# filodb/FiloDB

Measured on AMD Instinct MI355X. Metric: samples/sec scanned+aggregated, 1M series rate()[5m], higher is better.
Workload: dtype f64; 1 GPU; 1M counter series 1h@15s, rate()[5m] step=15s; series_per_gpu=1000000, windows=241, payload_bytes_per_gpu=886470800

## Files before the change

### filodb_amd/csrc/engine.hip

```cpp

#include <cstring>
#include <cstdio>
#include <cmath>
#include <vector>
#include <cstdlib>

#include "engine_internal.h"
#include "fast_desc.h"

struct fdb_engine {
  int device;
  hipStream_t stream;
  int32_t* dev_flag;
};

struct fdb_dataset {
  uint8_t* blob;
  uint64_t *ts_off, *val_off;
  int64_t *start_time, *end_time;
  int32_t *num_rows;
  int32_t *series_first, *series_nchunks, *group_ids;
  int32_t *series_by_group, *group_offsets;
  int32_t num_series;
  int64_t num_chunks;
  int64_t payload_bytes;
  int64_t total_samples;
  int max_group;
  int has_hist;
  int fast_ok;
  void* sums;
  uint64_t *max_off, *min_off;
  int has_mm;
  int has_sc;
  FdbFastDesc *fast_desc, *fast_desc_sc;
};

static DirSoA dir_of(const fdb_dataset_t* d, bool count_col = false) {
  return DirSoA{d->ts_off, count_col ? d->max_off : d->val_off,
                d->start_time, d->end_time, d->num_rows};
}

extern "C" fdb_engine_t* fdb_engine_create(int32_t device) {
  int count = 0;
  hipError_t e = hipGetDeviceCount(&count);
  if (e != hipSuccess || count == 0) {
    fdb_set_error("no HIP device present (hipGetDeviceCount: %s) — "
                  "filodb_amd has no CPU fallback", hipGetErrorString(e));
    return nullptr;
  }
  if (device < 0 || device >= count) { fdb_set_error("bad device %d", device); return nullptr; }
  HIP_CHECK_NULL(hipSetDevice(device));
  auto* eng = new fdb_engine();
  eng->device = device;
  if (hipStreamCreate(&eng->stream) != hipSuccess) {
    fdb_set_error("hipStreamCreate failed");
    delete eng;
    return nullptr;
  }
  if (hipMalloc(&eng->dev_flag, 4) != hipSuccess ||
      hipMemset(eng->dev_flag, 0, 4) != hipSuccess) {
    fdb_set_error("engine flag allocation failed");
    (void)hipStreamDestroy(eng->stream);
    delete eng;
    return nullptr;
  }
  return eng;
}
// ... 116 lines not shown
  };
  bool ok = upload_pad((void**)&d->blob, view.blob, (size_t)view.blob_len)
    && upload((void**)&d->ts_off, ts_off.data(), nc * 8)
    && upload((void**)&d->val_off, val_off.data(), nc * 8)
    && upload((void**)&d->start_time, st.data(), nc * 8)
    && upload((void**)&d->end_time, en.data(), nc * 8)
    && upload((void**)&d->num_rows, nr.data(), nc * 4)
    && upload((void**)&d->series_first, view.series_first, (size_t)view.num_series * 4)
    && upload((void**)&d->series_nchunks, view.series_nchunks, (size_t)view.num_series * 4)
    && upload((void**)&d->group_ids, view.group_ids, (size_t)view.num_series * 4)
    && upload((void**)&d->series_by_group, sbg.data(), sbg.size() * 4)
    && upload((void**)&d->group_offsets, goff.data(), goff.size() * 4)
    && upload((void**)&d->max_off, mx_off.data(), nc * 8)
    && upload((void**)&d->min_off, mn_off.data(), nc * 8);
  if (ok && d->fast_ok) {
    const int32_t ns = view.num_series;
    for (int col = 0; col < (d->has_sc ? 2 : 1) && d->fast_ok; col++) {
      const std::vector<uint64_t>& voff = col ? mx_off : val_off;
      std::vector<FdbFastDesc> desc((size_t)ns);
      int addressable = 1;
      #pragma omp parallel for schedule(static) reduction(&:addressable)
      for (int32_t sid = 0; sid < ns; sid++) {
        const int32_t c = view.series_first[sid];
        const bool has = view.series_nchunks[sid] >= 1;
        if (has && (((ts_off[c] | voff[c]) & 63) != 0 ||
                    ((ts_off[c] | voff[c]) >> 38) != 0)) {
          addressable = 0;
          continue;
        }
        fdb_build_fast_desc(view.blob, has ? ts_off[c] : 0, has ? voff[c] : 0,
                            has ? nr[c] : 0, &desc[(size_t)sid]);
      }
      if (!addressable) { d->fast_ok = 0; break; }
      ok = upload((void**)(col ? &d->fast_desc_sc : &d->fast_desc), desc.data(),
                  desc.size() * sizeof(FdbFastDesc));
      if (!ok) break;
    }
  }
  if (!ok) {
    fdb_set_error("device upload failed (out of HBM?)");
    fdb_dataset_destroy(d);
    return nullptr;
  }
  const char* fenv = getenv("FDB_FAST");
  const bool fast_off = fenv && atoi(fenv) == 0;
  if (has_scalar && (!d->fast_ok || fast_off)) {
    if (hipMalloc(&d->sums, (size_t)fdb_chunksum_bytes(nc)) != hipSuccess) {
      fdb_set_error("summary allocation failed (out of HBM?)");
      fdb_dataset_destroy(d);
      return nullptr;
    }
    if (fdb_launch_summaries(e->stream, d->blob, dir_of(d), nc, d->sums) != FDB_OK) {
      fdb_dataset_destroy(d);
      return nullptr;
    }
  }
  return d;
}

static bool fast_eligible(const fdb_dataset_t* d, const fdb_query_t* q) {
  const char* v = getenv("FDB_FAST");
  if (v && atoi(v) == 0) return false;
  return d->fast_ok && fdb_scan_supported(q->func_id) &&
         q->step > 0 && q->step < ((int64_t)1 << 31) && q->window >= 0;
}

static int32_t launch_scan(fdb_engine_t* e, const fdb_dataset_t* d, const fdb_query_t* q,
                           double* dev_out, double* dev_cnt, double* dev_sq,
                           bool count_col = false) {
  DirSoA dir = dir_of(d, count_col);
  int nw = fdb_num_windows(q);
  if (fast_eligible(d, q) && q->agg_id == AGG_NONE) {
    return fdb_launch_fast_scan(e->stream, d->blob,
                                count_col ? d->fast_desc_sc : d->fast_desc,
                                d->group_ids,
                                d->series_by_group, d->num_series,
                                q->start, q->step, q->window, nw,
                                q->func_id, AGG_NONE, 0,
                                dev_out, dev_cnt, dev_sq, q->_pad);
  }
  if (fdb_window_sample_supported(q->func_id)) {
    return fdb_launch_window_sample(e->stream, d->blob, dir, d->series_first,
                                    d->series_nchunks, d->num_series,
                                    q->start, q->step, q->window, nw,
                                    q->func_id, q->param, q->param2,
                                    dev_out, e->dev_flag);
  }
  if (!fdb_scan_supported(q->func_id)) {
    fdb_set_error("bad func_id %d", q->func_id);
    return FDB_ERR_BADARG;
  }
  if (!d->sums) {
    fdb_set_error("dataset has no chunk summaries (internal)");
    return FDB_ERR;
  }
  (void)dev_cnt; (void)dev_sq;
  return fdb_launch_stream_walk(e->stream, d->blob, dir, d->sums,
                                d->series_first, d->series_nchunks,
                                d->num_series, q->start, q->step, q->end,
                                q->window, nw, q->func_id, dev_out);
}

static int32_t check_windows(const fdb_query_t* q, const char* bad_nw, int* nw) {
  *nw = fdb_num_windows(q);
  if (*nw <= 0) { fdb_set_error("%s", bad_nw); return FDB_ERR_BADARG; }
  if (q->window > ((int64_t)1 << 33)) {
    fdb_set_error("window length > 2^33 ms (~99 days) unsupported");
// ... 50 lines not shown
  if (q->agg_id != AGG_NONE && !dev_cnt && !dev_cnt.alloc(out_len * 8))
    return alloc_failed("query");
  if (needs_sq) {
    if (partial) dev_sq.wrap(dev_out.get() + out_len);
    else if (!dev_sq.alloc(out_len * 8)) return alloc_failed("query");
  }
  HIP_CHECK(ev0.create());
  HIP_CHECK(ev1.create());

  const bool is_quant = q->agg_id == AGG_QUANTILE;
  if (is_quant && out_counts) {
    fdb_set_error("quantile aggregation has no partial (multi-shard) mode — "
                  "digest shipping is not implemented");
    return FDB_ERR_BADARG;
  }
  const char* fe = getenv("FDB_FUSED_GROUP");
  const bool fused = (fe && atoi(fe) == 1) && !is_quant &&
                     q->agg_id != AGG_NONE && !is_topk &&
                     nw <= 256 && fast_eligible(d, q);
  fdb_query_t qscan = *q;
  if (q->agg_id != AGG_NONE && !fused) {
    if (!per_grid.alloc((size_t)d->num_series * nw * 8)) return alloc_failed("query");
    qscan.agg_id = AGG_NONE;
  }

  auto run_once = [&]() -> int32_t {
    if (fused) {
      const bool mm = q->agg_id == AGG_MIN || q->agg_id == AGG_MAX;
      HIP_CHECK(hipMemsetAsync(dev_out.get(), mm ? 0xFF : 0, buf_len * 8, e->stream));
      HIP_CHECK(hipMemsetAsync(dev_cnt.get(), 0, out_len * 8, e->stream));
      if (dev_sq && !(needs_sq && partial))
        HIP_CHECK(hipMemsetAsync(dev_sq.get(), 0, out_len * 8, e->stream));
      return fdb_launch_fast_scan(
          e->stream, d->blob, d->fast_desc,
          d->group_ids, d->series_by_group, d->num_series,
          q->start, q->step, q->window, nw, q->func_id, q->agg_id,
          1, dev_out.get(), dev_cnt.get(), dev_sq.get(), q->_pad);
    }
    int32_t rc = launch_scan(e, d, &qscan, per_grid ? per_grid.get() : dev_out.get(),
                             per_grid ? nullptr : dev_cnt.get(), nullptr);
    if (rc != FDB_OK) return rc;
    if (is_topk)
      return fdb_launch_topk(e->stream, per_grid.get(), d->series_by_group,
                             d->group_offsets, q->num_groups, nw, kk,
                             q->agg_id == AGG_TOPK ? 1 : 0,
                             dev_out.get(), dev_cnt.get());
    if (is_quant)
      return fdb_launch_quantile_cells(e->stream, per_grid.get(),
                                       d->series_by_group, d->group_offsets,
                                       q->num_groups, nw, q->param, dev_out.get());
    if (q->agg_id != AGG_NONE)
      return fdb_launch_group_reduce(e->stream, per_grid.get(),
                                     d->series_by_group, d->group_offsets,
                                     q->num_groups, nw, q->agg_id,
                                     dev_out.get(), dev_cnt.get(), dev_sq.get());
    return FDB_OK;
  };

  int total_runs = warmup + iters;
  float ms_sum = 0;
  for (int it = 0; it < total_runs; it++) {
    bool timed = it >= warmup;
    if (timed) HIP_CHECK(hipEventRecord(ev0.get(), e->stream));
    if (int32_t rc = run_once()) return rc;
    if (timed) {
      HIP_CHECK(hipEventRecord(ev1.get(), e->stream));
      HIP_CHECK(hipEventSynchronize(ev1.get()));
// ... 223 lines not shown
```

### filodb_amd/csrc/engine_internal.h

```cpp
#ifndef FDB_ENGINE_INTERNAL_H
#define FDB_ENGINE_INTERNAL_H

#include <hip/hip_runtime.h>
#include <cstdint>

#include "chunk_format.h"
#include "scan_common.h"
#include "window_funcs.h"
#include "../../include/filodb_amd.h"

void fdb_set_error(const char* fmt, ...);
hipStream_t fdb_engine_stream(fdb_engine_t* e);

#define HIP_CHECK(expr) do { hipError_t _e = (expr); if (_e != hipSuccess) { \
  fdb_set_error("%s failed: %s", #expr, hipGetErrorString(_e)); return FDB_ERR; } } while (0)
#define HIP_CHECK_NULL(expr) do { hipError_t _e = (expr); if (_e != hipSuccess) { \
  fdb_set_error("%s failed: %s", #expr, hipGetErrorString(_e)); return nullptr; } } while (0)

template <typename T>
class DevPtr {
 public:
  DevPtr() = default;
  DevPtr(const DevPtr&) = delete;
  DevPtr& operator=(const DevPtr&) = delete;
// ... 22 lines not shown
  T* p_ = nullptr;
  bool owned_ = false;
};
using DevBuf = DevPtr<double>;

class DevEvent {
 public:
  DevEvent() = default;
  DevEvent(const DevEvent&) = delete;
  DevEvent& operator=(const DevEvent&) = delete;
  ~DevEvent() { if (ev_) (void)hipEventDestroy(ev_); }
  hipError_t create() { return hipEventCreate(&ev_); }
  hipEvent_t get() const { return ev_; }

 private:
  hipEvent_t ev_ = nullptr;
};

inline bool fdb_scan_supported(int func_id) {
  switch (func_id) {
    case FN_RATE: case FN_INCREASE: case FN_DELTA:
    case FN_SUM: case FN_COUNT: case FN_AVG: case FN_RATE_OVER_DELTA:
    case FN_MIN: case FN_MAX: case FN_STDDEV: case FN_STDVAR:
    case FN_CHANGES: case FN_LAST: case FN_PRESENT: case FN_TIMESTAMP:
    case FN_ZSCORE:
    case FN_IRATE: case FN_IDELTA: case FN_RESETS:
      return true;
    default:
      return false;
  }
}

struct FdbFastDesc;
int32_t fdb_launch_fast_scan(hipStream_t stream, const uint8_t* blob,
                             const FdbFastDesc* desc,
                             const int32_t* group_ids, const int32_t* series_by_group,
                             int num_series,
                             int64_t qstart, int64_t qstep, int64_t qwindow,
                             int num_windows, int func_id, int agg_id, int emit_group,
                             double* out, double* out_cnt, double* out_sq,
                             int phase_mask);

int32_t fdb_launch_summaries(hipStream_t stream, const uint8_t* blob, DirSoA dir,
                             int64_t num_chunks, void* sums);
int64_t fdb_chunksum_bytes(int64_t num_chunks);
int32_t fdb_launch_stream_walk(hipStream_t stream, const uint8_t* blob,
                               DirSoA dir, const void* sums,
                               const int32_t* series_first,
                               const int32_t* series_nchunks, int num_series,
                               int64_t qstart, int64_t qstep, int64_t qend,
                               int64_t qwindow, int num_windows, int func_id,
                               double* out);

bool fdb_window_sample_supported(int func_id);
int32_t fdb_launch_window_sample(hipStream_t stream, const uint8_t* blob,
                                 DirSoA dir, const int32_t* series_first,
                                 const int32_t* series_nchunks, int num_series,
                                 int64_t qstart, int64_t qstep, int64_t qwindow,
                                 int num_windows, int func_id, double param,
                                 double param2, double* out, int32_t* overflow);

int32_t fdb_launch_hist2(hipStream_t stream, const uint8_t* blob, DirSoA dir,
                         const uint64_t* max_off, const uint64_t* min_off,
                         const int32_t* series_first,
                         const int32_t* series_nchunks,
                         const int32_t* group_ids, int num_series,
                         int64_t qstart, int64_t qstep, int64_t qwindow,
                         int num_windows, int nb, int hfunc,
// ... 30 lines not shown
```

### filodb_amd/csrc/fast_desc.h

```cpp
#ifndef FDB_FAST_DESC_H
#define FDB_FAST_DESC_H

#include <cstdint>
#include <cstring>

#include "chunk_format.h"

enum { FDB_FD_CONST = 0,
       FDB_FD_PACKED = 1,
       FDB_FD_RAW64 = 2 };
enum { FDB_FD_SIGN = 1,
       FDB_FD_DROPPED = 2,
       FDB_FD_EXACT32 = 4 };

struct FdbFastDesc {
  uint32_t ts_unit;
  uint32_t val_unit;
  uint16_t n;
  uint8_t  ts_cls, ts_nbits;
  uint8_t  ts_flags, val_cls, val_nbits, val_flags;
  int64_t  ts0;
  int32_t  ts_base;
  int32_t  ts_slope;
  int64_t  val_init;
  int32_t  val_slope;
  uint32_t _pad[5];
};
static_assert(sizeof(FdbFastDesc) == 64, "one 64-byte scalar load per series");

struct FdbFdVec {
  int64_t init, first;
  int32_t slope, n;
  uint32_t payload;
  uint8_t cls, nbits, flags;
};

inline FdbFdVec fdb_fd_open(const uint8_t* p) {
  uint32_t h[8];
  memcpy(h, p, 32);
  FdbFdVec v;
  memset(&v, 0, sizeof(v));
  const uint16_t wf = (uint16_t)(h[1] & 0xffff);
  if (((h[1] >> 16) & FDB_DROP_MASK) != 0) v.flags |= FDB_FD_DROPPED;
  if (wf == FDB_WF_DDV) {
    v.cls = FDB_FD_PACKED;
    v.init = (int64_t)(((uint64_t)h[3] << 32) | h[2]);
    v.slope = (int32_t)h[4];
    const uint32_t w6 = h[6];
    v.nbits = (uint8_t)((w6 >> 16) & FDB_NBITS_MASK);
    if (((w6 >> 16) & FDB_SIGN_MASK) != 0) v.flags |= FDB_FD_SIGN;
    const int bitShift = (int)(w6 >> 24) & 0x3f;
    const int numBytes = (int)h[5];
    v.n = v.nbits
        ? ((numBytes - 4) * 8 + (bitShift != 0 ? bitShift - 8 : 0)) / v.nbits : 0;
    v.payload = FDB_DDV_OFF_INNER + FDB_PRIM_OFF_DATA;
    const bool sg = (v.flags & FDB_FD_SIGN) != 0;
    int64_t in0;
    switch (v.nbits) {
      case 32: in0 = (int32_t)h[7]; break;
// ... 7 lines not shown
    v.cls = FDB_FD_CONST;
    v.n = (int32_t)h[2];
    v.init = (int64_t)(((uint64_t)h[4] << 32) | h[3]);
    v.slope = (int32_t)h[5];
    v.first = v.init;
  } else {
    v.cls = FDB_FD_RAW64;
    v.n = ((int)h[0] - 4) / 8;
    v.nbits = 64;
    v.flags |= FDB_FD_SIGN;
    v.payload = FDB_PRIM_OFF_DATA;
    v.first = (int64_t)(((uint64_t)h[3] << 32) | h[2]);
  }
  return v;
}

inline int64_t fdb_fd_inner(const uint8_t* idata, int nbits, bool sign, int i) {
  switch (nbits) {
    case 32: { int32_t x; memcpy(&x, idata + 4 * (size_t)i, 4); return x; }
    case 16: { uint16_t u; memcpy(&u, idata + 2 * (size_t)i, 2);
               int32_t x = (int16_t)u; return sign ? x : (x & 0xffff); }
    case 8:  { int32_t x = (int8_t)idata[i]; return sign ? x : (x & 0xff); }
    case 4:  return (idata[i >> 1] >> ((i & 1) * 4)) & 0x0f;
    case 2:  return (idata[i >> 2] >> ((i & 3) * 2)) & 0x03;
  }
  return 0;
}

inline void fdb_build_fast_desc(const uint8_t* blob, uint64_t ts_off,
                                uint64_t val_off, int32_t num_rows,
                                FdbFastDesc* out) {
  FdbFastDesc d;
  memset(&d, 0, sizeof(d));
  if (num_rows > 0) {
    const FdbFdVec tv = fdb_fd_open(blob + ts_off);
    const FdbFdVec vv = fdb_fd_open(blob + val_off);
    d.ts_unit = (uint32_t)(ts_off >> 6);
    d.val_unit = (uint32_t)(val_off >> 6);
    d.ts_cls = tv.cls; d.ts_nbits = tv.nbits; d.ts_flags = tv.flags;
    d.val_cls = vv.cls; d.val_nbits = vv.nbits; d.val_flags = vv.flags;
    d.ts_slope = tv.slope;
    d.val_init = vv.init; d.val_slope = vv.slope;
    if (num_rows <= FDB_DEFAULT_MAX_ROWS && num_rows <= tv.n) {
      d.n = (uint16_t)num_rows;
      d.ts0 = tv.first;
      d.ts_base = (int32_t)(tv.init - tv.first);
      if (vv.cls == FDB_FD_PACKED && vv.n >= num_rows &&
          vv.init > -((int64_t)1 << 52) && vv.init < ((int64_t)1 << 52)) {
        const uint8_t* idata = blob + val_off + vv.payload;
        const bool sg = (vv.flags & FDB_FD_SIGN) != 0;
        bool fits = true;
        for (int i = 0; i < num_rows && fits; i++) {
          const int64_t off = (int64_t)vv.slope * i +
                              fdb_fd_inner(idata, vv.nbits, sg, i);
          fits = off >= INT32_MIN && off <= INT32_MAX;
        }
        if (fits) d.val_flags |= FDB_FD_EXACT32;
      }
    }
  }
  *out = d;
}

#endif
```

### filodb_amd/csrc/scan_fast.hip

```cpp

#include <cstddef>
#include <cstring>
#include <cmath>

#include "engine_internal.h"
#include "fast_desc.h"
#include "window_bounds.h"

#define FAST_TILE 256
#define FAST_WAVES 4
#define FAST_DROPS 32

#define K_RATE    0
#define K_PFX     1
#define K_PFX_SQ  2
#define K_MINMAX  3
#define K_CHANGES 4
#define K_LAST    5

template <int FUNC> struct FKind { static constexpr int v =
    (FUNC <= FN_DELTA) ? K_RATE :
    (FUNC == FN_SUM || FUNC == FN_AVG || FUNC == FN_COUNT ||
     FUNC == FN_RATE_OVER_DELTA) ? K_PFX :
    (FUNC == FN_STDDEV || FUNC == FN_STDVAR) ? K_PFX_SQ :
    (FUNC == FN_MIN || FUNC == FN_MAX) ? K_MINMAX :
    (FUNC == FN_CHANGES || FUNC == FN_RESETS) ? K_CHANGES :
    K_LAST; };

template <int KIND>
struct alignas(16) FWs {
  int32_t tso[FDB_DEFAULT_MAX_ROWS + 4];
  double  val[FDB_DEFAULT_MAX_ROWS];
  uint16_t cnt[(KIND == K_PFX || KIND == K_PFX_SQ || KIND == K_CHANGES)
                   ? FDB_DEFAULT_MAX_ROWS : 1];
  double  sq[KIND == K_PFX_SQ ? FDB_DEFAULT_MAX_ROWS : 1];
  double  grp[KIND == K_MINMAX ? (FDB_DEFAULT_MAX_ROWS + 7) / 8 : 1];
  int16_t dpos[KIND == K_RATE ? FAST_DROPS : 1];
  double  dcum[KIND == K_RATE ? FAST_DROPS : 1];
};

struct FDesc {
  uint32_t w[12];
  __device__ __forceinline__ int n() const { return (int)(w[2] & 0xffff); }
  __device__ __forceinline__ int ts_cls() const { return (int)((w[2] >> 16) & 0xff); }
  __device__ __forceinline__ int ts_nbits() const { return (int)(w[2] >> 24); }
  __device__ __forceinline__ int ts_flags() const { return (int)(w[3] & 0xff); }
  __device__ __forceinline__ int val_cls() const { return (int)((w[3] >> 8) & 0xff); }
  __device__ __forceinline__ int val_nbits() const { return (int)((w[3] >> 16) & 0xff); }
  __device__ __forceinline__ int val_flags() const { return (int)(w[3] >> 24); }
  __device__ __forceinline__ int64_t ts0() const {
    return (int64_t)(((uint64_t)w[5] << 32) | w[4]); }
  __device__ __forceinline__ int32_t ts_base() const { return (int32_t)w[6]; }
  __device__ __forceinline__ int32_t ts_slope() const { return (int32_t)w[7]; }
  __device__ __forceinline__ int64_t val_init() const {
    return (int64_t)(((uint64_t)w[9] << 32) | w[8]); }
  __device__ __forceinline__ int32_t val_slope() const { return (int32_t)w[10]; }
};
static_assert(offsetof(FdbFastDesc, n) == 8 && offsetof(FdbFastDesc, ts_flags) == 12 &&
              offsetof(FdbFastDesc, ts0) == 16 && offsetof(FdbFastDesc, ts_base) == 24 &&
              offsetof(FdbFastDesc, val_init) == 32 && offsetof(FdbFastDesc, val_slope) == 40,
              "FDesc's dword views follow FdbFastDesc's layout");

__device__ __forceinline__ FDesc fast_load_desc(const FdbFastDesc* desc, int s) {
  const uint4* p = reinterpret_cast<const uint4*>(desc + s);
  const uint4 a = p[0], b = p[1], c = p[2];
  return FDesc{{a.x, a.y, a.z, a.w, b.x, b.y, b.z, b.w, c.x, c.y, c.z, c.w}};
}

template <int KIND> constexpr bool needs_inv = KIND == K_PFX || KIND == K_PFX_SQ;
template <int KIND> constexpr int inv_entries =
    needs_inv<KIND> ? FDB_DEFAULT_MAX_ROWS + 2 : KIND == K_RATE ? FDB_RATE_RTAB : 0;

struct FastQuery {
  int64_t qstep, qwindow;
  double rate_scale, dur_ms;
  bool qw32;
  int rk_lim;
};

enum { PH_DECODE = 0, PH_META = 1, PH_BOUNDS = 2, PH_WINDOWS = 3 };
template <bool TIMED> struct FastTimer {
  uint64_t t[4] = {0, 0, 0, 0}, tt = 0;
  __device__ __forceinline__ void start() {
    if constexpr (TIMED) tt = __builtin_amdgcn_s_memtime();
  }
  __device__ __forceinline__ void lap(int phase) {
    if constexpr (TIMED) {
      const uint64_t now = __builtin_amdgcn_s_memtime();
      t[phase] += now - tt;
      tt = now;
    }
  }
  __device__ __forceinline__ void store(double* out, size_t gw, int lane) const {
    if constexpr (TIMED) {
      #pragma unroll
      for (int p = 0; p < 4; p++) if (lane == 0) out[gw * 4 + p] = (double)t[p];
    }
  }
};

struct FastChunk { int n; int64_t ts0; bool dropped; };

template <typename WS>
__device__ __forceinline__ FastChunk fast_decode(const FDesc& cd, const uint8_t* blob,
                                                 WS& ws, int lane) {
  const int n = cd.n();
  const int64_t ts0 = cd.ts0();
  const bool dropped = n > 0 && (cd.val_flags() & FDB_FD_DROPPED) != 0;
  if (n > 0) {
    int dl = lane;
    asm volatile("" : "+v"(dl));
    const uint8_t* tp = blob + ((size_t)cd.w[0] << 6);
    const uint8_t* vp = blob + ((size_t)cd.w[1] << 6);
    DVec tv;
    tv.wf = cd.ts_cls() == FDB_FD_PACKED ? FDB_WF_DDV
          : cd.ts_cls() == FDB_FD_CONST ? FDB_WF_DDV_CONST : FDB_WF_PRIM64;
    tv.idata = tp + (cd.ts_cls() == FDB_FD_PACKED
                         ? FDB_DDV_OFF_INNER + FDB_PRIM_OFF_DATA : FDB_PRIM_OFF_DATA);
    tv.init = ts0 + cd.ts_base();
    tv.slope = cd.ts_slope();
    tv.n = n; tv.nbits = (uint8_t)cd.ts_nbits();
    tv.sign = (cd.ts_flags() & FDB_FD_SIGN) != 0; tv.dropped = 0;
    d_decode_ts_offsets(tv, n, ts0, ws.tso, dl);
    const int vcls = cd.val_cls(), vbits = cd.val_nbits();
    const bool vsign = (cd.val_flags() & FDB_FD_SIGN) != 0;
    const bool exact32 = (cd.val_flags() & FDB_FD_EXACT32) != 0;
    const uint8_t* vdata = vp + FDB_DDV_OFF_INNER + FDB_PRIM_OFF_DATA;
    if (vcls == FDB_FD_PACKED && vbits == 8) {
      d_decode_val4<8>(vdata, vsign, cd.val_init(), cd.val_slope(), exact32,
                       n, ws.val, dl);
    } else if (vcls == FDB_FD_PACKED && vbits == 16) {
      d_decode_val4<16>(vdata, vsign, cd.val_init(), cd.val_slope(), exact32,
                        n, ws.val, dl);
    } else {
      DVec vv;
      vv.wf = vcls == FDB_FD_PACKED ? FDB_WF_DDV
            : vcls == FDB_FD_CONST ? FDB_WF_DDV_CONST : FDB_WF_PRIM64;
      vv.idata = vcls == FDB_FD_PACKED ? vdata : vp + FDB_PRIM_OFF_DATA;
      vv.init = cd.val_init(); vv.slope = cd.val_slope();
      vv.n = n; vv.nbits = (uint8_t)vbits; vv.sign = vsign; vv.dropped = dropped;
      d_decode_chunk<true>(vv, n, nullptr, ws.val, dl);
    }
  }
  return FastChunk{n, ts0, dropped};
}

template <int KIND, int FUNC, typename WS>
__device__ __forceinline__ ResetScan fast_meta(WS& ws, int n, bool dropped, int lane) {
  ResetScan rs;
  if constexpr (KIND == K_RATE) {
    if (dropped && n > 0) {
      for (int base = 0; base < n; base += 64) {
        int i = base + lane;
        double raw = (i < n) ? ws.val[i] : 0;
        double x = (i < n && !isnan(raw)) ? raw : 0;
        d_reset_scan_step<FAST_DROPS>(rs, i, i < n, x, lane, ws.dpos, ws.dcum);
// ... 24 lines not shown
      if constexpr (KIND == K_PFX_SQ) carry_sq += __shfl(sqs, 63);
    }
  }
  if constexpr (KIND == K_MINMAX) {
    for (int base = 0; base < n; base += 64) {
      int i = base + lane;
      double x = (i < n) ? ws.val[i] : NAN;
      #pragma unroll
      for (int off = 1; off < 8; off <<= 1)
        d_fold_mm<FUNC == FN_MIN>(x, __shfl_xor(x, off));
      if ((lane & 7) == 0 && i < n) ws.grp[i >> 3] = x;
    }
  }
  if constexpr (KIND == K_CHANGES) {
    int ccarry = 0;
    double carry_x = NAN;
    for (int base = 0; base < n; base += 64) {
      int i = base + lane;
      double x = (i < n) ? ws.val[i] : NAN;
      double px = __shfl_up(x, 1);
      if (lane == 0) px = carry_x;
      int ind = (i > 0 && i < n && d_pair_counts<FUNC == FN_RESETS>(x, px)) ? 1 : 0;
      int s = wave_incl_scan_i(ind, lane);
      if (i < n) ws.cnt[i] = (uint16_t)(ccarry + s);
      ccarry += __shfl(s, 63);
      carry_x = __shfl(x, 63);
    }
  }
  return rs;
}

struct WB { int s, e; int32_t t1, t2; };

template <bool SHARE>
struct FastBounds {
  const int32_t* tso;
  int n, lane, wshare;
  FastQuery q;
  FdbLin lin;
  int64_t Ae;
  int share_src;
  int s_prev;

  __device__ __forceinline__ FastBounds(const int32_t* tso_, int n_, int64_t Ae_,
                                        const FastQuery& q_, int wshare_, int lane_)
      : tso(tso_), n(n_), lane(lane_), wshare(wshare_), q(q_), Ae(Ae_),
        share_src(((lane_ - wshare_) & 63) << 2), s_prev(0) {
    const int32_t tlast = n > 0 ? tso[n - 1] : 0;
    lin.last = __builtin_amdgcn_readfirstlane(tlast);
    lin.inv_h = (n >= 2 && lin.last > 0) ? (float)(n - 1) / (float)lin.last : 0.0f;
    if constexpr (SHARE) {
      if (!fdb_windows_before_chunk(-1, q.qstep, Ae)) {
        int32_t unused;
        end_search(lane - 64, &unused, &s_prev);
      }
    }
  }
  __device__ __forceinline__ WB window_bounds(int w) const {
    WB b;
    const int64_t wEndOff = (int64_t)w * q.qstep - Ae;
    b.e = fdb_bound_e(tso, n, lin, wEndOff, &b.t2);
    b.s = fdb_bound_s(tso, n, lin, wEndOff - q.qwindow, &b.t1);
    return b;
  }
  __device__ __forceinline__ int end_search(int w, int32_t* t2, int* s_at_end) const {
    const int64_t x = (int64_t)w * q.qstep - Ae;
    int32_t t_next, unused;
    const int e = fdb_bound_core(tso, n, lin, x, t2, &t_next, nullptr);
    *s_at_end = fdb_bound_s_from_e(tso, n, lin, x, e, *t2, t_next, &unused);
    return e;
  }
  __device__ __forceinline__ WB shared_bounds(int w) {
    WB b;
    int s_cur;
    b.e = end_search(w, &b.t2, &s_cur);
    b.s = __builtin_amdgcn_ds_bpermute(share_src, lane < 64 - wshare ? s_cur : s_prev);
    s_prev = s_cur;
    b.t1 = tso[b.s];
    return b;
  }
  __device__ __forceinline__ WB calc_bounds(int k, int w, bool wok, int tn) {
    WB b = WB{1, -1, 0, 0};
    if constexpr (SHARE) {
      if (64 * k < tn) {
        const WB sb = shared_bounds(w);
        if (wok) b = sb;
      }
    } else if (wok) {
      b = window_bounds(w);
    }
    return b;
  }
};

template <int FUNC, typename WS>
__device__ __forceinline__ double fast_window_value(const WS& ws, const WB& wb, int w,
                                                    const FastChunk& ch,
                                                    const ResetScan& rs, int64_t Ae,
                                                    const FastQuery& q,
                                                    const double* inv_tab) {
  constexpr int KIND = FKind<FUNC>::v;
  const int s = wb.s, e = wb.e, n = ch.n;
  double res = NAN;
  if constexpr (KIND == K_RATE) {
    constexpr bool IS_COUNTER = (FUNC == FN_RATE || FUNC == FN_INCREASE);
    if (e > s) {
      const int t1 = wb.t1, t2 = wb.t2;
      if (t2 > t1) {
        double v1 = ws.val[s], v2 = ws.val[e];
        if (IS_COUNTER && ch.dropped) {
          if (isnan(v1)) v1 = 0;
          if (isnan(v2)) v2 = 0;
          auto row_at = [&](int j) { return ws.val[j]; };
          v1 += d_corr_at(ws.dpos, ws.dcum, rs.count, rs.dense, s, row_at);
          v2 += d_corr_at(ws.dpos, ws.dcum, rs.count, rs.dense, e, row_at);
        }
        const int64_t wEndOff = (int64_t)w * q.qstep - Ae;
        if (q.qw32)
// ... 18 lines not shown
      else if (pc > 0) {
        double qs = ws.sq[e] - (s ? ws.sq[s - 1] : 0.0);
        double inv = inv_tab[pc];
        double avg = ps * inv;
        double r = qs * inv - avg * avg;
        res = (FUNC == FN_STDDEV) ? sqrt(r) : r;
      }
    }
  } else if constexpr (KIND == K_MINMAX) {
    if (e >= s && e >= 0) {
      constexpr bool IS_MIN = (FUNC == FN_MIN);
      int ga = (s + 7) >> 3, gb = (e + 1) >> 3;
      if (ga < gb) {
        for (int i = s; i < ga * 8; i++) d_fold_mm<IS_MIN>(res, ws.val[i]);
        for (int g = ga; g < gb; g++) d_fold_mm<IS_MIN>(res, ws.grp[g]);
        for (int i = gb * 8; i <= e; i++) d_fold_mm<IS_MIN>(res, ws.val[i]);
      } else {
        for (int i = s; i <= e; i++) d_fold_mm<IS_MIN>(res, ws.val[i]);
      }
    }
  } else if constexpr (KIND == K_CHANGES) {
    if (e >= s && e >= 0) res = (double)((int)ws.cnt[e] - (int)ws.cnt[s]);
  } else if constexpr (FUNC == FN_TIMESTAMP) {
    if (e >= 0 && s < n) res = (double)(ch.ts0 + wb.t2) / 1000.0;
  } else if constexpr (FUNC == FN_PRESENT) {
    if (e >= s && e >= 0)
      d_present_at(ws.val[e], e, [&](int j) { return ws.val[j]; }, &res);
  } else if constexpr (FUNC == FN_LAST) {
    if (e >= s && e >= 0) res = ws.val[e];
  } else if constexpr (FUNC == FN_IRATE || FUNC == FN_IDELTA) {
    if (e > s) {
      const double last = ws.val[e], prev = ws.val[e - 1];
      if constexpr (FUNC == FN_IDELTA) res = last - prev;
      else res = d_irate_finish(last, prev, (double)(wb.t2 - ws.tso[e - 1]));
    }
  } else {
    if (e >= s && e >= 0) {
      double sm, sq;
      int pc;
      d_range_moments([&](int j) { return ws.val[j]; }, s, e, sm, sq, pc);
      res = d_zscore_finish(sm, sq, pc, ws.val[e]);
    }
  }
  return res;
}

struct FastGroupAcc {
  double accS[4] = {NAN, NAN, NAN, NAN}, accQ[4] = {}, accC[4] = {};
  int cur_grp = -1;
  __device__ __forceinline__ void clear() {
    #pragma unroll
    for (int k = 0; k < 4; k++) { accS[k] = NAN; accQ[k] = 0; accC[k] = 0; }
  }
  __device__ __forceinline__ void accumulate(int k, int agg_id, double res) {
    if (isnan(res)) return;
    accC[k] += 1.0;
    switch (agg_id) {
      case AGG_MIN: d_fold_mm<true>(accS[k], res); break;
      case AGG_MAX: d_fold_mm<false>(accS[k], res); break;
      case AGG_COUNT: case AGG_GROUP: break;
      case AGG_STDDEV: case AGG_STDVAR: accQ[k] += res * res; [[fallthrough]];
      default:
        accS[k] = isnan(accS[k]) ? res : accS[k] + res;
    }
  }
  __device__ __forceinline__ void flush(int lane, int num_windows, int agg_id,
                                        double* out, double* out_cnt, double* out_sq) {
    if (cur_grp < 0) return;
    #pragma unroll
    for (int k = 0; k < 4; k++) {
      int w = lane + 64 * k;
      if (w < num_windows && accC[k] > 0) {
        size_t cell = (size_t)cur_grp * num_windows + w;
        if (agg_id == AGG_MIN || agg_id == AGG_MAX)
          atomic_min_max_f64(&out[cell], accS[k], agg_id == AGG_MIN);
        else
          atomicAdd(&out[cell],
                    (agg_id == AGG_COUNT || agg_id == AGG_GROUP) ? accC[k] : accS[k]);
        atomicAdd(&out_cnt[cell], accC[k]);
        if (out_sq) atomicAdd(&out_sq[cell], accQ[k]);
      }
    }
    clear();
  }
};

template <int FUNC, int EMIT, int MINW, bool TIMED = false, bool SHARE = false>
__global__ __launch_bounds__(FAST_WAVES * 64, MINW)
void fast_scan_kernel(const uint8_t* __restrict__ blob,
                      const FdbFastDesc* __restrict__ desc,
                      const int32_t* __restrict__ group_ids,
                      const int32_t* __restrict__ sbg,
                      int num_series,
                      int64_t qstart, int64_t qstep, int64_t qwindow,
                      int num_windows, int agg_id,
                      double* __restrict__ out,
                      double* __restrict__ out_cnt,
                      double* __restrict__ out_sq,
                      int wshare)
{
  constexpr int KIND = FKind<FUNC>::v;
  __shared__ FWs<KIND> ws_all[FAST_WAVES];
  __shared__ double inv_tab[inv_entries<KIND> ? inv_entries<KIND> : 1];

  const int wave = __builtin_amdgcn_readfirstlane(threadIdx.x >> 6);
  const int lane = threadIdx.x & 63;
  FWs<KIND>& ws = ws_all[wave];

  if (inv_entries<KIND>) {
    for (int i = threadIdx.x; i < inv_entries<KIND>; i += FAST_WAVES * 64)
      inv_tab[i] = 1.0 / (double)i;
    __syncthreads();
  }

  const FastQuery q{qstep, qwindow, 1000.0 / (double)qwindow, (double)qwindow,
                    qwindow < ((int64_t)1 << 31),
                    qwindow <= (int64_t)FDB_RATE_RTAB_MAX_MS ? FDB_RATE_RTAB : 0};
  FastTimer<TIMED> timer;

  int pos0, pos1, pos_step;
  if (EMIT == 1) {
    const int gw = blockIdx.x * FAST_WAVES + wave;
    const int nwaves = gridDim.x * FAST_WAVES;
    const int slab = (num_series + nwaves - 1) / nwaves;
    pos0 = gw * slab;
    pos1 = min(num_series, pos0 + slab);
    pos_step = 1;
  } else {
    pos0 = blockIdx.x * FAST_WAVES + wave;
    pos1 = num_series;
    pos_step = gridDim.x * FAST_WAVES;
  }
  FastGroupAcc acc;

  for (int pos = pos0; pos < pos1; pos += pos_step) {
    timer.start();
    const int sid = __builtin_amdgcn_readfirstlane((EMIT == 1) ? sbg[pos] : pos);
    const FDesc cd = fast_load_desc(desc, sid);

    const FastChunk ch = fast_decode(cd, blob, ws, lane);
    d_lds_fence();
    timer.lap(PH_DECODE);

    const ResetScan rs = fast_meta<KIND, FUNC>(ws, ch.n, ch.dropped, lane);
    d_lds_fence();
    timer.lap(PH_META);

    if (EMIT == 1 && group_ids[sid] != acc.cur_grp) {
      acc.flush(lane, num_windows, agg_id, out, out_cnt, out_sq);
      acc.cur_grp = group_ids[sid];
    }

    FastBounds<SHARE> bnd(ws.tso, ch.n, ch.ts0 - qstart, q, wshare, lane);
    for (int tb = 0; tb < num_windows; tb += FAST_TILE) {
      const int tn = min(FAST_TILE, num_windows - tb);
      WB tbnd[TIMED ? 4 : 1];
      if constexpr (TIMED) {
        #pragma unroll
        for (int k = 0; k < 4; k++) {
          const int wi = lane + 64 * k;
          tbnd[k] = bnd.calc_bounds(k, tb + wi, wi < tn, tn);
          asm volatile("" :: "v"(tbnd[k].s ^ tbnd[k].e ^ tbnd[k].t1 ^ tbnd[k].t2));
        }
        timer.lap(PH_BOUNDS);
      }

      #pragma unroll
      for (int k = 0; k < 4; k++) {
        const int wi = lane + 64 * k;
        const int w = tb + wi;
        const bool wok = wi < tn;
        WB wb;
        if constexpr (TIMED) wb = tbnd[k];
        else wb = bnd.calc_bounds(k, w, wok, tn);
        const double res = fast_window_value<FUNC>(ws, wb, w, ch, rs, bnd.Ae, q, inv_tab);
        if constexpr (TIMED) asm volatile("" :: "v"(res));
        if (EMIT == 1) acc.accumulate(k, agg_id, res);
        else if (wok && !TIMED) out[(size_t)sid * num_windows + w] = res;
      }
      d_lds_fence();
      timer.lap(PH_WINDOWS);
    }
  }
  if (EMIT == 1) acc.flush(lane, num_windows, agg_id, out, out_cnt, out_sq);
  if (EMIT == 0) timer.store(out, (size_t)blockIdx.x * FAST_WAVES + wave, lane);
}

struct FastLaunch {
  int grid; hipStream_t stream;
  const uint8_t* blob; const FdbFastDesc* desc; const int32_t *group_ids, *sbg;
  int num_series; int64_t qstart, qstep, qwindow; int num_windows, agg_id;
  double *out, *out_cnt, *out_sq;
  int wshare;
  bool emit_group, timed;
};

template <int F, int EMIT, int MINW, bool TIMED>
static void launch_fast_as(const FastLaunch& a) {
  const auto kernel = a.wshare ? fast_scan_kernel<F, EMIT, MINW, TIMED, true>
                               : fast_scan_kernel<F, EMIT, MINW, TIMED, false>;
  hipLaunchKernelGGL(kernel, dim3(a.grid), dim3(FAST_WAVES * 64), 0, a.stream,
                     a.blob, a.desc, a.group_ids, a.sbg, a.num_series, a.qstart,
                     a.qstep, a.qwindow, a.num_windows, a.agg_id, a.out, a.out_cnt,
                     a.out_sq, a.wshare);
}
template <int F, int MINW>
static void launch_fast(const FastLaunch& a) {
  if (a.emit_group) return launch_fast_as<F, 1, 4, false>(a);
  if constexpr (F == FN_RATE || F == FN_AVG)
    if (a.timed) return launch_fast_as<F, 0, MINW, true>(a);
  launch_fast_as<F, 0, MINW, false>(a);
}

int32_t fdb_launch_fast_scan(hipStream_t stream, const uint8_t* blob,
                             const FdbFastDesc* desc,
                             const int32_t* group_ids, const int32_t* series_by_group,
                             int num_series,
                             int64_t qstart, int64_t qstep, int64_t qwindow,
                             int num_windows, int func_id, int agg_id, int emit_group,
                             double* out, double* out_cnt, double* out_sq,
                             int phase_mask) {
  int grid = (num_series + FAST_WAVES - 1) / FAST_WAVES;
  int cap = 16384;
  if (const char* g = getenv("FDB_GRID")) cap = atoi(g);
  if (cap > 0 && grid > cap) grid = cap;
  int wshare = 0;
  if (qstep > 0 && qwindow % qstep == 0 && qwindow / qstep >= 1 &&
      qwindow / qstep <= 64)
    wshare = (int)(qwindow / qstep);
  if (const char* s = getenv("FDB_WINDOW_SHARE")) { if (atoi(s) == 0) wshare = 0; }
  const FastLaunch a{grid, stream, blob, desc, group_ids, series_by_group,
                     num_series, qstart, qstep, qwindow, num_windows, agg_id,
                     out, out_cnt, out_sq, wshare, emit_group != 0,
                     (phase_mask & 8) != 0};
  switch (func_id) {
    case FN_RATE:            launch_fast<FN_RATE, 7>(a); break;
    case FN_INCREASE:        launch_fast<FN_INCREASE, 6>(a); break;
    case FN_DELTA:           launch_fast<FN_DELTA, 6>(a); break;
    case FN_SUM:             launch_fast<FN_SUM, 6>(a); break;
    case FN_COUNT:           launch_fast<FN_COUNT, 6>(a); break;
    case FN_AVG:             launch_fast<FN_AVG, 6>(a); break;
    case FN_RATE_OVER_DELTA: launch_fast<FN_RATE_OVER_DELTA, 6>(a); break;
    case FN_MIN:             launch_fast<FN_MIN, 6>(a); break;
    case FN_MAX:             launch_fast<FN_MAX, 6>(a); break;
    case FN_STDDEV:          launch_fast<FN_STDDEV, 3>(a); break;
    case FN_STDVAR:          launch_fast<FN_STDVAR, 3>(a); break;
    case FN_CHANGES:         launch_fast<FN_CHANGES, 6>(a); break;
    case FN_LAST:            launch_fast<FN_LAST, 6>(a); break;
    case FN_PRESENT:         launch_fast<FN_PRESENT, 6>(a); break;
    case FN_TIMESTAMP:       launch_fast<FN_TIMESTAMP, 6>(a); break;
    case FN_ZSCORE:          launch_fast<FN_ZSCORE, 6>(a); break;
    case FN_IRATE:           launch_fast<FN_IRATE, 6>(a); break;
    case FN_IDELTA:          launch_fast<FN_IDELTA, 6>(a); break;
    case FN_RESETS:          launch_fast<FN_RESETS, 6>(a); break;
    default:
      fdb_set_error("fast scan: unsupported func_id %d", func_id);
      return FDB_ERR_BADARG;
  }
  hipError_t e = hipGetLastError();
  if (e != hipSuccess) {
    fdb_set_error("fast_scan_kernel launch failed: %s", hipGetErrorString(e));
    return FDB_ERR;
  }
  return FDB_OK;
}
```

### filodb_amd/csrc/window_bounds.h

```cpp
#ifndef FDB_WINDOW_BOUNDS_H
#define FDB_WINDOW_BOUNDS_H

#include <cstdint>

#ifdef __HIPCC__
#define FDB_HD __host__ __device__
#else
#define FDB_HD
#endif

struct FdbLin {
  int32_t last;
  float inv_h;
};

FDB_HD inline FdbLin fdb_bounds_prepare(const int32_t* tso, int n) {
  FdbLin lin;
  lin.last = n > 0 ? tso[n - 1] : 0;
  lin.inv_h = (n >= 2 && lin.last > 0) ? (float)(n - 1) / (float)lin.last : 0.0f;
  return lin;
}

FDB_HD inline int fdb_bound_search(const int32_t* tso, int n, int32_t x) {
  int lo = 0, hi = n;
// ... 45 lines not shown
                              int32_t* t, int* residue = nullptr) {
  int32_t unused;
  return fdb_bound_core(tso, n, lin, x, t, &unused, residue);
}

FDB_HD inline int fdb_bound_s(const int32_t* tso, int n, FdbLin lin, int64_t y,
                              int32_t* t, int* residue = nullptr) {
  int32_t unused;
  return fdb_bound_core(tso, n, lin, y - 1, &unused, t, residue) + 1;
}

FDB_HD inline int fdb_bound_s_from_e(const int32_t* tso, int n, FdbLin lin,
                                     int64_t y, int E, int32_t t_e,
                                     int32_t t_next, int32_t* t1,
                                     int* residue = nullptr) {
  int s = E + 1;
  *t1 = t_next;
  if (E >= 0 && (int64_t)t_e == y) {
    if (E == 0 || tso[E - 1] < t_e) {
      s = E;
      *t1 = t_e;
    } else {
      s = fdb_bound_s(tso, n, lin, y, t1, residue);
    }
  }
  return s;
}

FDB_HD inline bool fdb_windows_before_chunk(int64_t w_last, int64_t qstep,
                                            int64_t Ae) {
  return w_last * qstep - Ae < 0;
}

#endif
```

Before: 177.8 billion samples/s.

## Add aligned-grid window bounds path when sample timestamps track query step

Computes per-series timestamp residual range at descriptor build time and stores it in previously padded descriptor bytes. At launch, a host-side sample of descriptors decides whether most series have one sample per step aligned to the query grid. If so, it selects a kernel variant that derives window start and end rows by direct index arithmetic with a single compare, replacing the interpolated search. This adds a kernel template variant, pads the timestamp buffer to allow neighbor reads at index -1, and costs a small per-series test in the bounds constructor with fallback to the existing path.

```diff
diff --git a/filodb_amd/csrc/engine.hip b/filodb_amd/csrc/engine.hip
--- a/filodb_amd/csrc/engine.hip
+++ b/filodb_amd/csrc/engine.hip
@@ -33,6 +33,8 @@
   int has_mm;
   int has_sc;
   FdbFastDesc *fast_desc, *fast_desc_sc;
+  FdbFastDesc fast_sample[2][FDB_FAST_SAMPLE];
+  int fast_nsample;
 };
 
 static DirSoA dir_of(const fdb_dataset_t* d, bool count_col = false) {
@@ -215,6 +217,9 @@
                             has ? nr[c] : 0, &desc[(size_t)sid]);
       }
       if (!addressable) { d->fast_ok = 0; break; }
+      d->fast_nsample = ns < FDB_FAST_SAMPLE ? ns : FDB_FAST_SAMPLE;
+      for (int k = 0; k < d->fast_nsample; k++)
+        d->fast_sample[col][k] = desc[(size_t)((int64_t)k * ns / d->fast_nsample)];
       ok = upload((void**)(col ? &d->fast_desc_sc : &d->fast_desc), desc.data(),
                   desc.size() * sizeof(FdbFastDesc));
       if (!ok) break;
@@ -256,6 +261,7 @@
   if (fast_eligible(d, q) && q->agg_id == AGG_NONE) {
     return fdb_launch_fast_scan(e->stream, d->blob,
                                 count_col ? d->fast_desc_sc : d->fast_desc,
+                                d->fast_sample[count_col ? 1 : 0], d->fast_nsample,
                                 d->group_ids,
                                 d->series_by_group, d->num_series,
                                 q->start, q->step, q->window, nw,
@@ -372,7 +378,7 @@
       if (dev_sq && !(needs_sq && partial))
         HIP_CHECK(hipMemsetAsync(dev_sq.get(), 0, out_len * 8, e->stream));
       return fdb_launch_fast_scan(
-          e->stream, d->blob, d->fast_desc,
+          e->stream, d->blob, d->fast_desc, d->fast_sample[0], d->fast_nsample,
           d->group_ids, d->series_by_group, d->num_series,
           q->start, q->step, q->window, nw, q->func_id, q->agg_id,
           1, dev_out.get(), dev_cnt.get(), dev_sq.get(), q->_pad);
diff --git a/filodb_amd/csrc/engine_internal.h b/filodb_amd/csrc/engine_internal.h
--- a/filodb_amd/csrc/engine_internal.h
+++ b/filodb_amd/csrc/engine_internal.h
@@ -78,8 +78,10 @@
 }
 
 struct FdbFastDesc;
+#define FDB_FAST_SAMPLE 256
 int32_t fdb_launch_fast_scan(hipStream_t stream, const uint8_t* blob,
                              const FdbFastDesc* desc,
+                             const FdbFastDesc* sample, int nsample,
                              const int32_t* group_ids, const int32_t* series_by_group,
                              int num_series,
                              int64_t qstart, int64_t qstep, int64_t qwindow,
diff --git a/filodb_amd/csrc/fast_desc.h b/filodb_amd/csrc/fast_desc.h
--- a/filodb_amd/csrc/fast_desc.h
+++ b/filodb_amd/csrc/fast_desc.h
@@ -24,7 +24,8 @@
   int32_t  ts_slope;
   int64_t  val_init;
   int32_t  val_slope;
-  uint32_t _pad[5];
+  int16_t  ts_rmin, ts_rmax;
+  uint32_t _pad[4];
 };
 static_assert(sizeof(FdbFastDesc) == 64, "one 64-byte scalar load per series");
 
@@ -98,6 +99,7 @@
                                 FdbFastDesc* out) {
   FdbFastDesc d;
   memset(&d, 0, sizeof(d));
+  d.ts_rmin = 1;
   if (num_rows > 0) {
     const FdbFdVec tv = fdb_fd_open(blob + ts_off);
     const FdbFdVec vv = fdb_fd_open(blob + val_off);
@@ -111,6 +113,25 @@
       d.n = (uint16_t)num_rows;
       d.ts0 = tv.first;
       d.ts_base = (int32_t)(tv.init - tv.first);
+      if (tv.cls != FDB_FD_RAW64 &&
+          tv.init - tv.first >= INT32_MIN && tv.init - tv.first <= INT32_MAX) {
+        const uint8_t* idata = blob + ts_off + tv.payload;
+        const bool sg = (tv.flags & FDB_FD_SIGN) != 0;
+        int64_t rmin = 0, rmax = 0;
+        bool fits = true;
+        for (int i = 0; i < num_rows && fits; i++) {
+          const int64_t in = tv.cls == FDB_FD_PACKED
+                                 ? fdb_fd_inner(idata, tv.nbits, sg, i) : 0;
+          const int64_t off = (tv.init - tv.first) + (int64_t)tv.slope * i + in;
+          if (i == 0 || in < rmin) rmin = in;
+          if (i == 0 || in > rmax) rmax = in;
+          fits = off >= 0 && off <= INT32_MAX;
+        }
+        if (fits && rmin >= INT16_MIN && rmax <= INT16_MAX) {
+          d.ts_rmin = (int16_t)rmin;
+          d.ts_rmax = (int16_t)rmax;
+        }
+      }
       if (vv.cls == FDB_FD_PACKED && vv.n >= num_rows &&
           vv.init > -((int64_t)1 << 52) && vv.init < ((int64_t)1 << 52)) {
         const uint8_t* idata = blob + val_off + vv.payload;
diff --git a/filodb_amd/csrc/scan_fast.hip b/filodb_amd/csrc/scan_fast.hip
--- a/filodb_amd/csrc/scan_fast.hip
+++ b/filodb_amd/csrc/scan_fast.hip
@@ -29,7 +29,9 @@
 
 template <int KIND>
 struct alignas(16) FWs {
-  int32_t tso[FDB_DEFAULT_MAX_ROWS + 4];
+  int32_t tsbuf[4 + FDB_DEFAULT_MAX_ROWS + 4];
+  __device__ __forceinline__ int32_t* tso() { return tsbuf + 4; }
+  __device__ __forceinline__ const int32_t* tso() const { return tsbuf + 4; }
   double  val[FDB_DEFAULT_MAX_ROWS];
   uint16_t cnt[(KIND == K_PFX || KIND == K_PFX_SQ || KIND == K_CHANGES)
                    ? FDB_DEFAULT_MAX_ROWS : 1];
@@ -55,10 +57,13 @@
   __device__ __forceinline__ int64_t val_init() const {
     return (int64_t)(((uint64_t)w[9] << 32) | w[8]); }
   __device__ __forceinline__ int32_t val_slope() const { return (int32_t)w[10]; }
+  __device__ __forceinline__ int32_t ts_rmin() const { return (int32_t)(int16_t)(w[11] & 0xffff); }
+  __device__ __forceinline__ int32_t ts_rmax() const { return (int32_t)w[11] >> 16; }
 };
 static_assert(offsetof(FdbFastDesc, n) == 8 && offsetof(FdbFastDesc, ts_flags) == 12 &&
               offsetof(FdbFastDesc, ts0) == 16 && offsetof(FdbFastDesc, ts_base) == 24 &&
-              offsetof(FdbFastDesc, val_init) == 32 && offsetof(FdbFastDesc, val_slope) == 40,
+              offsetof(FdbFastDesc, val_init) == 32 && offsetof(FdbFastDesc, val_slope) == 40 &&
+              offsetof(FdbFastDesc, ts_rmin) == 44 && offsetof(FdbFastDesc, ts_rmax) == 46,
               "FDesc's dword views follow FdbFastDesc's layout");
 
 __device__ __forceinline__ FDesc fast_load_desc(const FdbFastDesc* desc, int s) {
@@ -76,6 +81,7 @@
   double rate_scale, dur_ms;
   bool qw32;
   int rk_lim;
+  float inv_qstep;
 };
 
 enum { PH_DECODE = 0, PH_META = 1, PH_BOUNDS = 2, PH_WINDOWS = 3 };
@@ -121,7 +127,7 @@
     tv.slope = cd.ts_slope();
     tv.n = n; tv.nbits = (uint8_t)cd.ts_nbits();
     tv.sign = (cd.ts_flags() & FDB_FD_SIGN) != 0; tv.dropped = 0;
-    d_decode_ts_offsets(tv, n, ts0, ws.tso, dl);
+    d_decode_ts_offsets(tv, n, ts0, ws.tso(), dl);
     const int vcls = cd.val_cls(), vbits = cd.val_nbits();
     const bool vsign = (cd.val_flags() & FDB_FD_SIGN) != 0;
     const bool exact32 = (cd.val_flags() & FDB_FD_EXACT32) != 0;
@@ -212,7 +218,7 @@
 
 struct WB { int s, e; int32_t t1, t2; };
 
-template <bool SHARE>
+template <bool SHARE, bool ALIGNED>
 struct FastBounds {
   const int32_t* tso;
   int n, lane, wshare;
@@ -222,10 +228,20 @@
   int share_src;
   int s_prev;
 
+  FdbAligned al;
+
   __device__ __forceinline__ FastBounds(const int32_t* tso_, int n_, int64_t Ae_,
-                                        const FastQuery& q_, int wshare_, int lane_)
-      : tso(tso_), n(n_), lane(lane_), wshare(wshare_), q(q_), Ae(Ae_),
-        share_src(((lane_ - wshare_) & 63) << 2), s_prev(0) {
+                                        const FastQuery& q_, int wshare_, int lane_,
+                                        const FDesc& cd, int nw)
+      : tso(tso_), n(n_), lane(lane_), wshare(wshare_), q(q_), lin{0, 0.0f}, Ae(Ae_),
+        share_src(((lane_ - wshare_) & 63) << 2), s_prev(0), al{false, 0, 0} {
+    if constexpr (ALIGNED) {
+      const int32_t k0 = __builtin_amdgcn_readfirstlane(fdb_aligned_guess(
+          cd.ts_base(), cd.ts_rmin(), cd.ts_rmax(), Ae, q.inv_qstep));
+      al = fdb_aligned_test(n, cd.ts_base(), cd.ts_slope(), cd.ts_rmin(),
+                            cd.ts_rmax(), Ae, q.qstep, wshare, nw, k0);
+      if (al.ok) return;
+    }
     const int32_t tlast = n > 0 ? tso[n - 1] : 0;
     lin.last = __builtin_amdgcn_readfirstlane(tlast);
     lin.inv_h = (n >= 2 && lin.last > 0) ? (float)(n - 1) / (float)lin.last : 0.0f;
@@ -259,11 +275,20 @@
     b.t1 = tso[b.s];
     return b;
   }
+  __device__ __forceinline__ WB aligned_bounds(int w) const {
+    WB b;
+    const int32_t x = (int32_t)((uint32_t)al.x0 + (uint32_t)w * (uint32_t)q.qstep);
+    const int32_t y = (int32_t)((uint32_t)x - (uint32_t)q.qwindow);
+    fdb_aligned_bounds(tso, n, al.k0, w, wshare, x, y, &b.e, &b.s, &b.t1, &b.t2);
+    return b;
+  }
   __device__ __forceinline__ WB calc_bounds(int k, int w, bool wok, int tn) {
     WB b = WB{1, -1, 0, 0};
     if constexpr (SHARE) {
       if (64 * k < tn) {
-        const WB sb = shared_bounds(w);
+        WB sb;
+        if (ALIGNED && al.ok) sb = aligned_bounds(w);
+        else sb = shared_bounds(w);
         if (wok) b = sb;
       }
     } else if (wok) {
@@ -348,7 +373,7 @@
     if (e > s) {
       const double last = ws.val[e], prev = ws.val[e - 1];
       if constexpr (FUNC == FN_IDELTA) res = last - prev;
-      else res = d_irate_finish(last, prev, (double)(wb.t2 - ws.tso[e - 1]));
+      else res = d_irate_finish(last, prev, (double)(wb.t2 - ws.tso()[e - 1]));
     }
   } else {
     if (e >= s && e >= 0) {
@@ -401,7 +426,8 @@
   }
 };
 
-template <int FUNC, int EMIT, int MINW, bool TIMED = false, bool SHARE = false>
+template <int FUNC, int EMIT, int MINW, bool TIMED = false, bool SHARE = false,
+          bool ALIGNED = false>
 __global__ __launch_bounds__(FAST_WAVES * 64, MINW)
 void fast_scan_kernel(const uint8_t* __restrict__ blob,
                       const FdbFastDesc* __restrict__ desc,
@@ -431,7 +457,8 @@
 
   const FastQuery q{qstep, qwindow, 1000.0 / (double)qwindow, (double)qwindow,
                     qwindow < ((int64_t)1 << 31),
-                    qwindow <= (int64_t)FDB_RATE_RTAB_MAX_MS ? FDB_RATE_RTAB : 0};
+                    qwindow <= (int64_t)FDB_RATE_RTAB_MAX_MS ? FDB_RATE_RTAB : 0,
+                    1.0f / (float)qstep};
   FastTimer<TIMED> timer;
 
   int pos0, pos1, pos_step;
@@ -467,7 +494,8 @@
       acc.cur_grp = group_ids[sid];
     }
 
-    FastBounds<SHARE> bnd(ws.tso, ch.n, ch.ts0 - qstart, q, wshare, lane);
+    FastBounds<SHARE, ALIGNED> bnd(ws.tso(), ch.n, ch.ts0 - qstart, q, wshare, lane,
+                                   cd, num_windows);
     for (int tb = 0; tb < num_windows; tb += FAST_TILE) {
       const int tn = min(FAST_TILE, num_windows - tb);
       WB tbnd[TIMED ? 4 : 1];
@@ -508,13 +536,16 @@
   int num_series; int64_t qstart, qstep, qwindow; int num_windows, agg_id;
   double *out, *out_cnt, *out_sq;
   int wshare;
+  bool aligned;
   bool emit_group, timed;
 };
 
 template <int F, int EMIT, int MINW, bool TIMED>
 static void launch_fast_as(const FastLaunch& a) {
-  const auto kernel = a.wshare ? fast_scan_kernel<F, EMIT, MINW, TIMED, true>
-                               : fast_scan_kernel<F, EMIT, MINW, TIMED, false>;
+  const auto kernel =
+      !a.wshare ? fast_scan_kernel<F, EMIT, MINW, TIMED, false, false>
+      : a.aligned ? fast_scan_kernel<F, EMIT, MINW, TIMED, true, true>
+                  : fast_scan_kernel<F, EMIT, MINW, TIMED, true, false>;
   hipLaunchKernelGGL(kernel, dim3(a.grid), dim3(FAST_WAVES * 64), 0, a.stream,
                      a.blob, a.desc, a.group_ids, a.sbg, a.num_series, a.qstart,
                      a.qstep, a.qwindow, a.num_windows, a.agg_id, a.out, a.out_cnt,
@@ -528,8 +559,12 @@
   launch_fast_as<F, 0, MINW, false>(a);
 }
 
+static int32_t g_last_aligned = 0;
+extern "C" int32_t fdb_debug_last_fast_aligned(void) { return g_last_aligned; }
+
 int32_t fdb_launch_fast_scan(hipStream_t stream, const uint8_t* blob,
                              const FdbFastDesc* desc,
+                             const FdbFastDesc* sample, int nsample,
                              const int32_t* group_ids, const int32_t* series_by_group,
                              int num_series,
                              int64_t qstart, int64_t qstep, int64_t qwindow,
@@ -545,9 +580,26 @@
       qwindow / qstep <= 64)
     wshare = (int)(qwindow / qstep);
   if (const char* s = getenv("FDB_WINDOW_SHARE")) { if (atoi(s) == 0) wshare = 0; }
+  int sampled = 0, eligible = 0;
+  if (wshare) {
+    const float inv_q = 1.0f / (float)qstep;
+    for (int i = 0; i < nsample; i++) {
+      const FdbFastDesc& d = sample[i];
+      if (d.n == 0) continue;
+      sampled++;
+      const int64_t A = d.ts0 - qstart;
+      const int32_t k0 = fdb_aligned_guess(d.ts_base, d.ts_rmin, d.ts_rmax, A, inv_q);
+      if (fdb_aligned_test(d.n, d.ts_base, d.ts_slope, d.ts_rmin, d.ts_rmax, A, qstep,
+                           wshare, num_windows, k0).ok)
+        eligible++;
+    }
+  }
+  bool aligned = eligible > 0 && 4 * eligible >= sampled;
+  if (const char* s = getenv("FDB_ALIGNED")) { if (atoi(s) == 0) aligned = false; }
+  g_last_aligned = aligned ? eligible : 0;
   const FastLaunch a{grid, stream, blob, desc, group_ids, series_by_group,
                      num_series, qstart, qstep, qwindow, num_windows, agg_id,
-                     out, out_cnt, out_sq, wshare, emit_group != 0,
+                     out, out_cnt, out_sq, wshare, aligned, emit_group != 0,
                      (phase_mask & 8) != 0};
   switch (func_id) {
     case FN_RATE:            launch_fast<FN_RATE, 7>(a); break;
diff --git a/filodb_amd/csrc/window_bounds.h b/filodb_amd/csrc/window_bounds.h
--- a/filodb_amd/csrc/window_bounds.h
+++ b/filodb_amd/csrc/window_bounds.h
@@ -101,4 +101,65 @@
   return w_last * qstep - Ae < 0;
 }
 
+struct FdbAligned {
+  bool ok;
+  int32_t k0;
+  int32_t x0;
+};
+
+FDB_HD inline int32_t fdb_aligned_guess(int32_t ts_base, int32_t rmin, int32_t rmax,
+                                        int64_t A, float inv_q) {
+  const float k = __builtin_rintf(
+      ((float)(A + ts_base) + 0.5f * (float)(rmin + rmax)) * inv_q);
+  return (k > -1.0e9f && k < 1.0e9f) ? (int32_t)k : INT32_MIN;
+}
+
+FDB_HD inline FdbAligned fdb_aligned_test(int n, int32_t ts_base, int32_t ts_slope,
+                                          int32_t rmin, int32_t rmax, int64_t A,
+                                          int64_t q, int64_t m, int64_t nw,
+                                          int32_t k0) {
+  FdbAligned al{false, k0, (int32_t)(uint32_t)(0 - (uint64_t)A)};
+  const int64_t lim = (int64_t)1 << 40;
+  if (n < 1 || rmin > rmax || k0 == INT32_MIN || q < 1 || q >= ((int64_t)1 << 30) ||
+      m < 1 || m > 64 || nw < 1 || nw >= ((int64_t)1 << 30) || A <= -lim || A >= lim)
+    return al;
+  const int64_t x_first = -m * q - A, x_last = (nw - 1) * q - A;
+  if (x_first < INT32_MIN || x_last > INT32_MAX) return al;
+  const int64_t d = (int64_t)ts_slope - q, dn = (int64_t)(n - 1) * d;
+  const int64_t C0 = (int64_t)ts_base + A - (int64_t)k0 * q;
+  const int64_t lo = C0 + rmin + (dn < 0 ? dn : 0);
+  const int64_t hi = C0 + rmax + (dn > 0 ? dn : 0);
+  al.ok = lo > -q && hi < q;
+  return al;
+}
+
+FDB_HD inline int fdb_aligned_row(int n, int32_t k0, int w) {
+  const int j = w - k0;
+  return j < 0 ? 0 : (j > n - 1 ? n - 1 : j);
+}
+
+FDB_HD inline int fdb_aligned_e_pick(int j, int32_t below, int32_t at, int32_t x,
+                                     int32_t* t2) {
+  const bool gt = at > x;
+  *t2 = gt ? below : at;
+  return j - (int)gt;
+}
+
+FDB_HD inline int fdb_aligned_s_pick(int j, int32_t at, int32_t above, int32_t y,
+                                     int32_t* t1) {
+  const bool lt = at < y;
+  *t1 = lt ? above : at;
+  return j + (int)lt;
+}
+
+FDB_HD inline void fdb_aligned_bounds(const int32_t* tso, int n, int32_t k0, int w,
+                                      int m, int32_t x, int32_t y, int* e, int* s,
+                                      int32_t* t1, int32_t* t2) {
+  const int je = fdb_aligned_row(n, k0, w), js = fdb_aligned_row(n, k0, w - m);
+  const int32_t e_below = tso[je - 1], e_at = tso[je];
+  const int32_t s_at = tso[js], s_above = tso[js + 1];
+  *e = fdb_aligned_e_pick(je, e_below, e_at, x, t2);
+  *s = fdb_aligned_s_pick(js, s_at, s_above, y, t1);
+}
+
 #endif
```

Measured after the change: 197.4 billion samples/s, median of 6. 1.11x the previous value.
